# uio-bmi/compairr

Measured on AMD Instinct MI355X. Metric: query sequences/sec for --matrix d=1, 10M-vs-10M CDR3aa, higher is better.
Workload: dtype u64; 1 GPU; synthetic 10M-vs-10M CDR3aa, d=1 substitutions only, V/J matched; queries_total=10000000, queries_this_gpu=10000000, reference_sequences=10000000, matrix_checksum=fc9769626ca2bcf2c84e8473864b8853

## Files before the change

### compairr_amd/csrc/compairr_hip.hip

```cpp
#include "context.h"
#include "kernels_sliced.h"
#include "kernels_rows.h"
#include "kernels_pairs2.h"
#include "select.h"

#include <algorithm>
#include <cmath>
#include <cstdio>
#include <cstdlib>
#include <cstring>
#include <new>
#include <mutex>
#include <string>
#include <thread>
#include <vector>

using namespace cmpr;

std::string &cmpr_create_error()
{
  static thread_local std::string e;
  return e;
}

// ... 225 lines not shown
  invalidate_plan(c);
  c->zob.release();
  c->res2.release(); c->off2.release(); c->cnt2.release();
  c->page_tab.release();
  c->bloom.release(); c->v2.release(); c->j2.release(); c->rep2.release();
  c->rec2.release(); c->voff2.release(); c->bmap2.release();
  for (RefPart &p : c->xparts)
    p.release();
  c->xparts.clear();
  c->stats_acc.release();
  c->tiles.release(); c->qres.release(); c->qv.release(); c->qj.release(); c->qgh.release();
  c->qlen.release(); c->qck.release();
  c->qhins.release(); c->qhdel.release(); c->items.release(); c->cpk.release(); c->qpk.release(); c->slice_items.release(); c->qrec.release();
  c->matrix.release(); c->matrix_f64.release();
  c->pos_buf.release(); c->pos_ctr.release(); c->d_ctab.release(); c->chunks.release(); c->tile_refs.release(); c->small_tiles.release();
  for (uint32_t i = 0; i < cmpr_context::TIME_RING; i++) {
    if (c->ring_k0[i]) (void)hipEventDestroy(c->ring_k0[i]);
    if (c->ring_km[i]) (void)hipEventDestroy(c->ring_km[i]);
    if (c->ring_k1[i]) (void)hipEventDestroy(c->ring_k1[i]);
  }
  if (c->ev_stop) (void)hipEventDestroy(c->ev_stop);
  if (c->ev_usage) (void)hipEventDestroy(c->ev_usage);
  if (c->d_usage) (void)hipFree(c->d_usage);
  if (c->h_usage) (void)hipHostFree(c->h_usage);
  c->arena_a.release();
  c->arena_b.release();
  if (c->stage_host) (void)hipHostFree(c->stage_host);
  if (c->h_sizes) (void)hipHostFree(c->h_sizes);
  for (uint32_t i = 0; i < cmpr_context::NCOPY_EV; i++)
    if (c->ev_copy[i]) (void)hipEventDestroy(c->ev_copy[i]);
// ... 107 lines not shown
    if (value < 1 || value > 2)
      return fail(c, CMPR_EINVAL, "d2_buffers must be 1 or 2");
    if (c->have_ref)
      return fail(c, CMPR_ESTATE, "set d2_buffers before cmpr_set_reference");
    c->d2_buffers = value;
  } else if (n == "chunk_deal") {
    if (value < 0 || value > 1)
      return fail(c, CMPR_EINVAL, "chunk_deal must be 0 (static) or 1 (by a counter)");
    c->chunk_deal = value;
  } else if (n == "narrow_upload") {
    if (value < -1 || value > 1)
      return fail(c, CMPR_EINVAL, "narrow_upload must be -1 (auto), 0 or 1");
    c->narrow_upload = value;
    affects_plan = false;
  } else if (n == "item_wg" || n == "layout_recompute" || n == "layout_timing" || n == "layout_zob_lds" ||
             n == "record_tiles") {
    if (value < 0 || value > (n == "record_tiles" ? 2 : 1))
      return fail(c, CMPR_EINVAL, n + (n == "record_tiles" ? " must be 0, 1 or 2" : " must be 0 or 1"));
    if (n == "record_tiles" && c->have_q)
      return fail(c, CMPR_ESTATE, "set record_tiles before cmpr_set_queries");
    (n == "item_wg" ? c->item_wg : n == "layout_recompute" ? c->layout_recompute :
     n == "layout_zob_lds" ? c->layout_zob_lds : n == "record_tiles" ? c->record_tiles : c->layout_timing) = value;
    affects_plan = false;
  } else if (n == "assume_never_overflows") {
    c->force_no_redo = value != 0;
    c->usage_pending = false;
    affects_plan = false;
  } else if (n == "resolve_blocks_per_cu") {
    if (value < 1 || value > 8)
      return fail(c, CMPR_EINVAL, "resolve_blocks_per_cu must be 1..8");
    c->resolve_blocks_per_cu = value;
  } else if (n == "pos_segments") {
    if (value < 1 || value > 256 || (value & (value - 1)))
      return fail(c, CMPR_EINVAL, "pos_segments must be a power of two, 1..256");
    if (c->have_q)
      return fail(c, CMPR_ESTATE, "set pos_segments before cmpr_set_queries");
    c->pos_segments = value;
// ... 98 lines not shown
  else if (n == "slice_words_log2") *value = c->sliced && c->have_ref ? (int64_t)c->geom.words_log2 : c->slice_words_log2;
  else if (n == "slice_bytes") *value = !c->sliced ? 0 : c->rows ? (int64_t)c->geom.rw_words * ROW_WORD_BYTES : (int64_t)8 << c->geom.words_log2;
  else if (n == "passes") *value = c->npasses;
  else if (n == "chunk_tiles") *value = c->chunk_tiles > 0 ? c->chunk_tiles : 8 * c->waves_per_block;
  else if (n == "waves_per_block") *value = c->plan.valid ? (int64_t)c->plan.nw : c->waves_per_block;
  else if (n == "narrow_upload") *value = c->narrow_upload;
  else if (n == "d2_buffers") *value = c->have_ref && c->d2pairs ? (int64_t)c->geom.nbuf : c->d2_buffers;
  else if (n == "d2_pairs") *value = c->have_ref ? (c->d2pairs ? 1 : 0) : c->d2_pairs;
  else if (n == "chunk_deal") *value = c->chunk_deal;
  else if (n == "layout_upload_us") *value = (int64_t)(c->layout_upload_ms * 1e3);
  else if (n == "layout_tail_us") *value = (int64_t)(c->layout_tail_ms * 1e3);
  else if (n == "layout_total_us") *value = (int64_t)(c->layout_total_ms * 1e3);
  else if (n == "item_wg") *value = c->item_wg;
  else if (n == "layout_recompute") *value = c->layout_recompute;
  else if (n == "layout_timing") *value = c->layout_timing;
  else if (n == "record_tiles") *value = c->have_q ? (c->rec_tiles ? (c->rec_hash ? 1 : 2) : 0) : c->record_tiles;
  else if (n == "layout_keys_us") *value = (int64_t)(c->layout_kernel_ms[0] * 1e3);
  else if (n == "layout_sizes_us") *value = (int64_t)(c->layout_kernel_ms[1] * 1e3);
  else if (n == "layout_scatter_us") *value = (int64_t)(c->layout_kernel_ms[2] * 1e3);
  else if (n == "layout_tiles_us") *value = (int64_t)(c->layout_kernel_ms[3] * 1e3);
  else if (n == "layout_order_us") *value = (int64_t)(c->layout_kernel_ms[4] * 1e3);
  else if (n == "never_overflows") *value = c->never_overflows ? 1 : 0;
  else if (n == "debug") *value = c->debug;
  else if (n == "heavy_threshold") *value = c->heavy_threshold;
  else if (n == "class_anchor") *value = c->sliced && c->have_ref ? (int64_t)c->geom.c0 : c->class_anchor;
  else if (n == "heavy_buckets") {
    *value = 0;
    if (c->sliced && c->have_ref)
      for (uint32_t w = 0; w < HEAVY_WORDS; w++)
        *value += __builtin_popcount(c->ctab[c->geom.off_hv + w]);
// ... 226 lines not shown

static int retire_queries(cmpr_context *c)
{
  HIP_TRY(c, hipSetDevice(c->device));
  if (c->events_valid)
    c->pending_launch = c->ev_k1;
  c->have_q = false;
  c->usage_pending = c->never_overflows = false;
  c->last_without_redo = false;
  c->events_valid = false;
  c->calls = 0;
  invalidate_plan(c);
  return CMPR_OK;
}

int cmpr_settle_previous_launch(cmpr_context *c)
{
  int rc;
  if ((rc = cmpr_wait_previous_launch(c)))
    return rc;
  if (c->async_unchecked || c->async_overflowed) {
    unsigned long long sticky = 0;
    HIP_TRY(c, hipMemcpy(&sticky, c->d_usage + 1, sizeof sticky, hipMemcpyDeviceToHost));
    const bool bad = sticky != 0 || c->async_overflowed;
    if (sticky)
      HIP_TRY(c, hipMemset(c->d_usage + 1, 0, sizeof sticky));
    c->async_unchecked = c->async_overflowed = false;
    if (bad)
      return fail(c, CMPR_ESTATE, "positives buffer overflowed in a launch without redo pass on the previous "
                                  "query set: its result was invalid (cmpr_get_stats was not asked); repeat "
                                  "the call to set the new queries");
  }
  return CMPR_OK;
// ... 11 lines not shown
    std::string why;
    rc = validate_view(c->opt, src.view, why, src.kind == LayoutSource::DEVICE);
    if (rc)
      return fail(c, rc, why);
  } else {
    if (src.nrec && !src.d_records)
      return fail(c, CMPR_EINVAL, "d_records is NULL");
    if (src.nrec && src.n_rep == 0)
      return fail(c, CMPR_EINVAL, "n_repertoires is 0");
    if (src.nrec >= 0xffffffc0ull || src.n_total > 0xffffffffull)
      return fail(c, CMPR_EUNSUPPORTED, "more than 2^32-64 sequences in one set");
  }
  if ((rc = retire_queries(c)))
    return rc;

  src.finish = [c]() -> int {
  int rc;
  const size_t cells = (size_t)c->R1 * c->R2;
  if ((rc = dev_reserve(c, c->matrix, cells))) return rc;
  if (is_f64_score(c->opt)) {
    if ((rc = dev_reserve(c, c->matrix_f64, cells))) return rc;
  } else {
    c->matrix_f64.release();
  }
  {
    const uint64_t per_query = c->rows && c->opt.differences == 2 ? 32 : 4;
    const uint64_t total = c->pos_capacity > 0 ? (uint64_t)c->pos_capacity
                                               : (1u << 20) + per_query * c->n1 /
                                                     (c->routed ? 1ull : (uint64_t)c->work_shard_count);
    const uint64_t S = (uint64_t)c->pos_segments;
    c->pos_cap = (total + S - 1) / S;
    if ((rc = dev_reserve(c, c->pos_buf, S * (c->pos_cap + WAVE)))) return rc;
    if ((rc = dev_reserve(c, c->pos_ctr, 2 * ctr_block_words(S)))) return rc;
    c->ctr_clean = false;
    use_counter_block(c, 0);
    const size_t cells = (size_t)c->R1 * c->R2;
    c->part_stride = (uint32_t)((cells <= PART_CELLS_MAX && !is_f64_score(c->opt) ? cells : 0) + STAT_COUNT);
    if ((rc = dev_reserve(c, c->part, (size_t)NPART * c->part_stride))) return rc;
    HIP_TRY(c, hipMemsetAsync(c->part.p, 0, (size_t)NPART * c->part_stride * sizeof(unsigned long long),
                              c->stream));
  }
  return CMPR_OK;
  };

  if ((rc = cmpr_layout_queries(c, src)))
    return rc;
  if ((rc = make_plan(c))) return rc;
  c->have_q = true;
  return CMPR_OK;
}


static __global__ void __launch_bounds__(WAVE)
sum_part_stats_kernel(const unsigned long long *stats, const unsigned long long *overflow,
                      const unsigned long long *stats2, unsigned long long *acc)
{
  const uint32_t k = threadIdx.x;
// ... 224 lines not shown
  if (!S.will_launch) {
    HIP_TRY(c, hipMemsetAsync(c->ctr_other, 0, S.ctr_blk * sizeof(unsigned long long), st));
    if (c->nparts > 1)
      HIP_TRY(c, hipMemsetAsync(c->stats_acc.p, 0, STAT_COUNT * sizeof(unsigned long long), st));
    if (ev_km)
      HIP_TRY(c, hipEventRecord(ev_km, st));
    c->launches = 0;
    return CMPR_OK;
  }
  const uint32_t np = c->nparts;
  if (np > 1)
    HIP_TRY(c, hipMemsetAsync(c->stats_acc.p, 0, STAT_COUNT * sizeof(unsigned long long), st));
  const bool resolve_pass = S.deferred && !(c->debug & DBG_SKIP_RESOLVE);
  unsigned long long *sticky = (S.redo_kind && !a.with_redo) ? c->d_usage + 1 : nullptr;
  uint32_t launches = 0;
  for (uint32_t k = 0; k < np; k++) {
    ProbeParams P = S.P;
    if (k > 0) {
      use_counter_block(c, c->ctr_cur == c->pos_ctr.p ? 1 : 0);
      const RefPart &rp = c->xparts[k - 1];
      P.bloom = rp.bloom.p;
      P.dir_mask = (uint32_t)(rp.slots - 1);
      P.bmap = S.P.bmap ? rp.bmap.p : nullptr;
      P.rec2 = rp.rec.p;
    }
    P.matrix = a.d_out;
    P.tile_counter = c->d_tile_counter;
    P.deal_ctr = c->d_deal;
    P.stats = c->d_stats;
    P.pair_q = c->pair_q;
    P.pair_h = c->pair_h;
    P.pair_count = c->pair_count;
    P.pair_cap = c->pair_cap;
    if (S.deferred)
      P.pos_ctr = c->ctr_cur;
    if (c->rows && S.deferred)
      P.overflow = c->d_overflow;
    hipLaunchKernelGGL(S.fn, dim3(S.grid), dim3(S.nw * WAVE), S.lds, st, P);
    HIP_TRY(c, hipGetLastError());
    launches += 1;
    if (ev_km && k + 1 == np)
      HIP_TRY(c, hipEventRecord(ev_km, st));
    if (a.track_usage && k == 0)
      HIP_TRY(c, hipMemsetAsync(c->d_usage, 0, sizeof(unsigned long long), st));
    auto reduce_partials = [&]() {
      hipLaunchKernelGGL(reduce_partials_kernel, dim3(P.part_stride), dim3(NPART), 0, st, P,
                         P.part_cells, S.reduce_writes ? 1u : 0u, c->ctr_other,
                         (uint32_t)S.ctr_blk, a.track_usage ? c->d_usage : nullptr, sticky);
    };
    if (!resolve_pass) {
      reduce_partials();
      HIP_TRY(c, hipGetLastError());
    } else {
      hipLaunchKernelGGL(S.rfn, dim3(S.rgrid), dim3(BLOCK_THREADS), S.rlds, st, P);
      reduce_partials();
      HIP_TRY(c, hipGetLastError());
      launches += 1;
      if (a.track_usage && k + 1 == np) {
        HIP_TRY(c, hipMemcpyAsync(c->h_usage, c->d_usage, sizeof(unsigned long long),
// ... 617 lines not shown
```

### compairr_amd/csrc/context.h

```cpp
#ifndef COMPAIRR_AMD_CONTEXT_H
#define COMPAIRR_AMD_CONTEXT_H

#include "../../include/compairr_hip.h"
#include "kernels.h"

#include "select.h"

#include <functional>
#include <map>
#include <set>
#include <string>
#include <vector>

struct SplitMix64 {
  uint64_t s;
  explicit SplitMix64(uint64_t seed) : s(seed) {}
  uint64_t next()
  {
    uint64_t z = (s += 0x9e3779b97f4a7c15ull);
    z = (z ^ (z >> 30)) * 0xbf58476d1ce4e5b9ull;
    z = (z ^ (z >> 27)) * 0x94d049bb133111ebull;
    return z ^ (z >> 31);
  }
};
// ... 40 lines not shown
  uint32_t grid = 0, nw = 0, rgrid = 0;
  size_t   lds = 0, rlds = 0;
};

struct LayoutSource {
  enum Kind { HOST, DEVICE, RECORDS } kind = HOST;
  const cmpr_set_view *view = nullptr;
  const void   *d_records = nullptr;
  uint64_t      nrec = 0;
  uint32_t      n_rep = 0;
  uint64_t      n_total = 0;
  const double *totals = nullptr;
  bool          route = false;
  uint64_t      first_index = 0;
  std::function<int()> finish;
};

struct RouteState {
  bool     valid = false;
  uint64_t n = 0, first_index = 0, total_records = 0;
  uint32_t n_dest = 0, record_bytes = 0;
  unsigned long long counts[64] = {};
  std::vector<double> rep_totals;
  const uint8_t  *res = nullptr;
  const uint64_t *off = nullptr, *cnt = nullptr;
  const uint32_t *v = nullptr, *j = nullptr, *rep = nullptr;
  const uint32_t *mask_lo = nullptr, *mask_hi = nullptr;
  unsigned long long *dest = nullptr;
};

// ... 60 lines not shown
  int64_t debug = 0;
  int64_t slice_words_log2 = -1;
  uint32_t chunk_cap = 0;

  bool                  sliced = false;
  bool                  rows = false;
  uint32_t              npasses = 1;
  SliceGeom             geom{};
  std::vector<uint32_t> ctab;
  DevBuf<uint32_t>      d_ctab;
  DevBuf<uint32_t>      page_tab;
  uint64_t              page_slices = 0;
  DevBuf<Chunk>         chunks;
  DevBuf<cmpr::TileRef> tile_refs;
  DevBuf<uint32_t>      small_tiles;
  uint32_t              nsmall = 0;
  uint32_t              nchunks = 0;

  uint32_t          zpos = 0;
  DevBuf<uint64_t>  zob;

  bool              have_ref = false;
  uint64_t          n2 = 0;
  uint32_t          R2 = 0, longest2 = 0;
  DevBuf<uint8_t>   res2;
  DevBuf<uint64_t>  off2, cnt2, bloom;
  DevBuf<uint32_t>  v2, j2, rep2;
  DevBuf<uint32_t>  bmap2;
  DevBuf<unsigned char> rec2;
  DevBuf<uint32_t>  voff2;
  uint64_t          slots = 0, bloom_words = 0;
  int64_t           part_buckets_log2 = 30;
  uint32_t          nparts = 1;
  uint64_t          part0_n = 0;
  std::vector<RefPart> xparts;
  DevBuf<unsigned long long> stats_acc;

  bool              have_q = false;
  bool              routed = false;
  RouteState        route;
  uint64_t          n1 = 0;
  uint32_t          R1 = 0, ntiles = 0;
  DevBuf<TileDesc>  tiles;
  uint32_t          nmain_tiles = 0;
  DevBuf<uint32_t>  qres, qv, qj;
  DevBuf<uint64_t>  qgh;
  DevBuf<uint64_t>  qhins, qhdel;
  DevBuf<uint16_t>  qlen;
  DevBuf<uint32_t>  qck;
  DevBuf<cmpr::QueryRec> qrec;
  DevBuf<cmpr::ItemRec> items;
  DevBuf<uint32_t>  slice_items;
  DevBuf<cmpr::ResPack> cpk;
  DevBuf<cmpr::ResPack> qpk;
  bool              d2pairs = false;
  int64_t           d2_pairs = -1;
  int64_t           d2_buffers = 1;
  uint64_t          algorithmic_bytes = 0;
  double            max_cell_bound = 0;
  std::vector<double> tot1, tot2;

  DevBuf<unsigned long long> matrix;
  DevBuf<double>             matrix_f64;
  DevBuf<PosEntry>           pos_buf;
  DevBuf<unsigned long long> pos_ctr;
  unsigned long long        *ctr_cur = nullptr, *ctr_other = nullptr;
  bool                       ctr_clean = false;
// ... 5 lines not shown
  bool                       last_without_redo = false;
  bool                       force_no_redo = false;
  bool                       async_unchecked = false, async_overflowed = false;
  hipStream_t                last_stream = nullptr;
  bool                       have_last_stream = false;
  DevArena                   arena_a, arena_b;
  void                      *stage_host = nullptr;
  size_t                     stage_host_bytes = 0;
  int64_t                    narrow_upload = -1;
  hipStream_t                copy_stream = nullptr;
  static const uint32_t      NCOPY_EV = 4;
  hipEvent_t                 ev_copy[NCOPY_EV] = {};
  double                     layout_upload_ms = 0, layout_tail_ms = 0, layout_total_ms = 0;
  int64_t                    item_wg = 1, layout_recompute = 1, layout_timing = 0;
  int64_t                    layout_zob_lds = 1;
  int64_t                    record_tiles = 1;
  bool                       rec_tiles = false;
  bool                       rec_hash = false;
  std::map<std::pair<const void *, size_t>, int> occupancy_seen;
  std::set<std::pair<const void *, size_t>>      lds_raised;
  void                      *h_sizes = nullptr;
  size_t                     h_sizes_bytes = 0;
  hipEvent_t                 ev_layout[6] = {};
  uint32_t                   layout_marks = 0;
  float                      layout_kernel_ms[5] = {};
  StepPlan                   plan;
  unsigned long long        *d_stats = nullptr;
  uint32_t                  *d_tile_counter = nullptr;
  unsigned long long        *d_overflow = nullptr, *d_stats2 = nullptr;
  uint32_t                  *d_tile_counter2 = nullptr;
  unsigned long long        *d_deal = nullptr;
  DevBuf<unsigned long long> part;
  uint32_t                   part_stride = 0;
  const void                *attr_fn2 = nullptr;
  size_t                     attr_lds2 = 0;
  uint64_t                   pos_cap = 0;
  uint32_t                   launches = 0;
  const void                *attr_fn = nullptr;
  size_t                     attr_lds = 0;
// ... 42 lines not shown
  HIP_TRY(c, hipMalloc((void **)&b.p, n * sizeof(T)));
  b.n = n;
  b.cap = n;
  return CMPR_OK;
}

inline int cmpr_wait_previous_launch(cmpr_context *c)
{
  if (c->pending_launch) {
    HIP_TRY(c, hipEventSynchronize(c->pending_launch));
    c->pending_launch = nullptr;
  }
  return CMPR_OK;
}

int cmpr_settle_previous_launch(cmpr_context *c);

template <typename T>
int dev_reserve(cmpr_context *c, DevBuf<T> &b, size_t n)
{
  if (n == 0)
    n = 1;
  if (b.p && b.cap >= n) {
    b.n = n;
    return CMPR_OK;
  }
  b.release();
  const size_t want = n + n / 16;
  HIP_TRY(c, hipMalloc((void **)&b.p, want * sizeof(T)));
  b.n = n;
  b.cap = want;
// ... 61 lines not shown
```

### compairr_amd/csrc/query_layout.hip

```cpp
#include "context.h"
#include "kernels_sliced.h"

#include <hipcub/hipcub.hpp>

#include <algorithm>
#include <atomic>
#include <chrono>
#include <cstdio>
#include <cstdlib>
#include <cstring>
#include <thread>

using namespace cmpr;

namespace {

constexpr uint32_t MAXP = 1 + MAX_CLASS_RES;
constexpr uint32_t FOREIGN_SLICES_LOG2 = 12;

enum : uint32_t { VERR_OFFSETS = 1, VERR_LONG = 2, VERR_REP = 3, VERR_GENE = 4, VERR_COUNT = 5,
                  VERR_RESIDUE = 6, VERR_TOO_LONG = 7, VERR_OFFSETS0 = 8 };

struct SliceTot {
  uint32_t tiles, chunks, small, list;
// ... 1888 lines not shown
        (void)hipStreamSynchronize(c->copy_stream);
        (void)hipStreamSynchronize(c->stream);
      }
    }
  } quiesce{c};
  const cmpr_set_view *const s = src.view;
  const bool from_host = src.kind == LayoutSource::HOST;
  const bool from_records = src.kind == LayoutSource::RECORDS;
  const bool routing = src.route;
  const uint32_t A = (uint32_t)c->opt.alphabet_size;
  const uint32_t Lcap = c->zpos - EXTRA_POSITIONS;
  const uint64_t n = from_records ? src.nrec : s->n;
  const uint32_t n_rep = from_records ? src.n_rep : s->n_repertoires;
  const uint32_t record_bytes = route_record_bytes(Lcap);
  c->route.valid = false;
  uint64_t total = 0;
  if (from_host) {
    total = n ? s->offsets[n] : 0;
  } else if (from_records) {
    total = n * (uint64_t)Lcap;
  }
  const bool total_on_device = src.kind == LayoutSource::DEVICE && n > 0;
  if (n > 0x7fffffffull)
    return fail(c, CMPR_EUNSUPPORTED, "more than 2^31-1 sequences in one set");
  if (!total_on_device && total > 0xffffull * n)
    return fail(c, CMPR_EINVAL, verr_message(VERR_OFFSETS));
  const bool soa_in_arena = src.kind != LayoutSource::DEVICE || n == 0;
  if (!routing) {
    c->n1 = n;
    c->R1 = c->opt.existence ? (uint32_t)(from_records ? src.n_total : n) : n_rep;
// ... 209 lines not shown
    b = 0;
    (void)hipcub::DeviceScan::ExclusiveSum(nullptr, b, (uint32_t *)nullptr, (uint32_t *)nullptr, big, c->stream);
    cub_bytes = std::max(cub_bytes, b);
    b = 0;
    (void)sum64(nullptr, b, nullptr, nullptr, big, c->stream);
    cub_bytes = std::max(cub_bytes, b);
    if (narrow || from_records) {
      hipcub::TransformInputIterator<unsigned long long, Len16To64, const uint16_t *> it(nullptr, Len16To64());
      b = 0;
      (void)hipcub::DeviceScan::ExclusiveScan(nullptr, b, it, (unsigned long long *)nullptr, hipcub::Sum(),
                                              0ull, (int)(n + 1), c->stream);
      cub_bytes = std::max(cub_bytes, b);
    }
  }
  const size_t o_cub = cut.take(cub_bytes + 256);
  if (!(c->arena_a.base && c->arena_a.cap >= cut.used) && (rc = cmpr_wait_previous_launch(c)))
    return rc;
  if ((rc = arena_fit(c, c->arena_a, cut.used))) return rc;
  const auto t_arena_a = std::chrono::steady_clock::now();
  char *const base = c->arena_a.base;
  auto at = [&](size_t off) -> char * { return base + off; };
  HIP_TRY(c, hipMemsetAsync(base, 0, zero_bytes, c->stream));

  QL Q;
  memset(&Q, 0, sizeof Q);
  if (soa_in_arena) {
    Q.res = (const uint8_t *)at(o_res);
    Q.off = (const uint64_t *)at(o_off);
    Q.v = c->opt.ignore_genes ? nullptr : (const uint32_t *)at(o_v);
    Q.j = c->opt.ignore_genes ? nullptr : (const uint32_t *)at(o_j);
    Q.rep = (const uint32_t *)at(o_rep);
    Q.cnt = c->opt.ignore_counts ? nullptr : (const uint64_t *)at(o_cnt);
// ... 438 lines not shown
  }
  const uint64_t cslots = hsums[0], class_chunks = hsums[1];
  if (ntiles * WAVE >= 0xffffffffull)
    return fail(c, CMPR_EUNSUPPORTED, "too many query tiles");
  if (res_words + 9 * WAVE >= 0xffffffffull || cslots + WAVE >= 0xffffffffull)
    return fail(c, CMPR_EUNSUPPORTED, "query set too large for 32-bit residue positions");
  const uint64_t main_chunks = nchunks, main_list = nlist;
  const uint64_t sib_list = hsums[2], sib_chunks = hsums[3];
  nchunks += sib_chunks;
  nlist += sib_list;
  Q.cchunk0 = (uint32_t)nchunks;
  nchunks += class_chunks;
  if (nchunks >= 0x7fffffffull || nlist >= 0xffffffffull)
    return fail(c, CMPR_EUNSUPPORTED, "too many chunks");

  if ((rc = cmpr_settle_previous_launch(c)))
    return rc;

  const size_t slots = (size_t)ntiles * WAVE;
  size_t sort_bytes = 0, small_sort_bytes = 0;
  if (nchunks)
    (void)hipcub::DeviceRadixSort::SortPairsDescending(nullptr, sort_bytes, (uint32_t *)nullptr, (uint32_t *)nullptr,
                                                       (uint32_t *)nullptr, (uint32_t *)nullptr, (int)nchunks, 0, 32,
                                                       c->stream);
  if (nsmall)
    (void)hipcub::DeviceRadixSort::SortPairsDescending(nullptr, small_sort_bytes, (uint32_t *)nullptr,
                                                       (uint32_t *)nullptr, (uint32_t *)nullptr, (uint32_t *)nullptr,
                                                       (int)nsmall, 0, 17, c->stream);
  ArenaCut cb;
  const size_t o_aux = cb.take(std::max<size_t>(Q.recompute ? 1 : slots, 1) * sizeof(QAux));
  const size_t o_chunks_u = cb.take((size_t)nchunks * sizeof(Chunk));
  const size_t o_wk = cb.take(((size_t)nchunks + 1) * sizeof(uint32_t));
  const size_t o_wk2 = cb.take((size_t)nchunks * sizeof(uint32_t));
  const size_t o_ix = cb.take((size_t)nchunks * sizeof(uint32_t));
  const size_t o_ix2 = cb.take((size_t)nchunks * sizeof(uint32_t));
  const size_t o_sort = cb.take(sort_bytes + 256);
  const size_t o_ln = cb.take((size_t)nsmall * sizeof(uint32_t));
  const size_t o_ln2 = cb.take((size_t)nsmall * sizeof(uint32_t));
  const size_t o_sout = cb.take((size_t)nsmall * sizeof(uint32_t));
  const size_t o_ssort = cb.take(small_sort_bytes + 256);
  if ((rc = arena_fit(c, c->arena_b, cb.used))) return rc;
  char *const bb = c->arena_b.base;
  Chunk *const chunks_unsorted = (Chunk *)(bb + o_chunks_u);
  Q.aux = (QAux *)(bb + o_aux);

  c->ntiles = (uint32_t)ntiles;
  c->nchunks = (uint32_t)nchunks;
  c->nsmall = (uint32_t)nsmall;
  if ((rc = dev_reserve(c, c->tiles, (size_t)ntiles))) return rc;
  if ((rc = dev_reserve(c, c->chunks, (size_t)nchunks))) return rc;
  if ((rc = dev_reserve(c, c->tile_refs, (size_t)nlist))) return rc;
  if ((rc = dev_reserve(c, c->small_tiles, (size_t)nsmall))) return rc;
  if ((rc = dev_reserve(c, c->qres, (size_t)res_words + 9 * WAVE))) return rc;
  if ((rc = dev_reserve(c, c->qlen, slots))) return rc;
  if ((rc = dev_reserve(c, c->qrec, slots))) return rc;
  HIP_TRY(c, hipMemsetAsync(c->qres.p + res_words, 0, 9 * WAVE * sizeof(uint32_t), c->stream));
  if (!c->opt.ignore_genes && !c->rows) {
    if ((rc = dev_reserve(c, c->qv, slots))) return rc;
    if ((rc = dev_reserve(c, c->qj, slots))) return rc;
  } else {
    c->qv.release();
    c->qj.release();
  }
  if (!c->opt.ignore_genes || c->rows || (!c->sliced && c->opt.differences == 0)) {
    if ((rc = dev_reserve(c, c->qgh, slots))) return rc;
  } else {
    c->qgh.release();
  }
  if (c->rows) {
    if ((rc = dev_reserve(c, c->qck, slots))) return rc;
  } else {
    c->qck.release();
  }
  if (c->d2pairs) {
    if ((rc = dev_reserve(c, c->qpk, slots))) return rc;
  } else {
    c->qpk.release();
  }
  if (c->rows && c->opt.indels) {
    if ((rc = dev_reserve(c, c->qhins, slots))) return rc;
    if ((rc = dev_reserve(c, c->qhdel, slots))) return rc;
  } else {
    c->qhins.release();
    c->qhdel.release();
  }
  bool pad_items = false;
  if (ngroups) {
    const size_t ni = (size_t)cslots + WAVE;
    if ((rc = dev_reserve(c, c->items, ni))) return rc;
    pad_items = true;
    if (sub2_items) {
      if ((rc = dev_reserve(c, c->cpk, ni))) return rc;
      if ((rc = dev_reserve(c, c->slice_items, 2 * (size_t)nslices_real))) return rc;
      HIP_TRY(c, hipMemsetAsync(c->slice_items.p, 0, 2 * (size_t)nslices_real * sizeof(uint32_t), c->stream));
    } else if (c->d2pairs) {
      if ((rc = dev_reserve(c, c->cpk, ni))) return rc;
      c->slice_items.release();
    } else {
      c->cpk.release();
      c->slice_items.release();
    }
  } else {
    c->items.release();
    c->cpk.release();
    c->slice_items.release();
  }
  const auto t_reserved = std::chrono::steady_clock::now();
  Q.tiles = c->tiles.p;
  Q.chunks = chunks_unsorted;
  Q.tile_refs = c->tile_refs.p;
  Q.small_tiles = c->small_tiles.p;
  Q.cpk = c->cpk.p;
  Q.qpk = c->qpk.p;
  Q.slice_items = (uint2 *)c->slice_items.p;
  Q.qres = c->qres.p; Q.qv = c->qv.p; Q.qj = c->qj.p;
  Q.qck = c->qck.p; Q.qgh = c->qgh.p; Q.qhins = c->qhins.p;
  Q.qhdel = c->qhdel.p; Q.qlen = c->qlen.p; Q.qrec = c->qrec.p;
  Q.items = c->items.p;

  if (pad_items) {
    hipLaunchKernelGGL(item_padding_kernel, dim3(blocks_for(std::max<uint64_t>(ncs, WAVE))), dim3(256), 0, c->stream, Q,
                       cpad, (uint32_t)cslots);
    HIP_TRY(c, hipGetLastError());
  }
  hipLaunchKernelGGL(slices_kernel<1>, dim3((uint32_t)((nslices + SLICES_WG - 1) / SLICES_WG)), dim3(SLICES_WG),
                     slices_lds, c->stream, Q, 0u, slices_lds ? 1u : 0u);
  HIP_TRY(c, hipGetLastError());
  LAYOUT_MARK(2);
  if (n) {
    for (const Range &g : ranges) {
      hipLaunchKernelGGL(scatter_fn, dim3(g.grid), dim3(LAYOUT_WG), scatter_lds, c->stream, Q, g.q0, g.q1, g.row0);
      HIP_TRY(c, hipGetLastError());
    }
  }
  LAYOUT_MARK(3);
  c->rec_tiles = rows_rec;
  c->rec_hash = c->rec_tiles && rec_hash;
  if (ntiles && !c->rec_tiles) {
    const size_t fill_lds = Q.recompute ? (zob_lds ? zob_words * sizeof(uint64_t) : 0) + ctab_bytes : 0;
    const int fo = occupancy_of(c, (const void *)fill_tiles_kernel, 256, fill_lds);
    const uint32_t fgrid = (uint32_t)std::min<uint64_t>((ntiles + 3) / 4, (uint64_t)c->cus * (uint64_t)std::max(fo, 1));
    hipLaunchKernelGGL(fill_tiles_kernel, dim3(fgrid), dim3(256), fill_lds, c->stream, Q, (uint32_t)ntiles);
    HIP_TRY(c, hipGetLastError());
  }
  LAYOUT_MARK(4);
  if (ngroups) {
    hipLaunchKernelGGL(class_chunks_kernel, dim3(blocks_for(ncs)), dim3(256), 0, c->stream, Q);
    HIP_TRY(c, hipGetLastError());
  }
  if (indel_passes) {
    hipLaunchKernelGGL(sibling_fill_kernel, dim3(blocks_for(G)), dim3(256), 0, c->stream, Q, G,
                       sib_lpre, sib_fill, (uint32_t)main_list);
    HIP_TRY(c, hipGetLastError());
    hipLaunchKernelGGL(sibling_write_chunks_kernel, dim3(blocks_for(2 * nslices)), dim3(256), 0,
                       c->stream, Q, sib_cnt, sib_lpre, sib_cpre, (uint32_t)main_list,
                       (uint32_t)main_chunks);
    HIP_TRY(c, hipGetLastError());
  }

  const bool select_share = wstep > 1 && !place_mine;
  if (nchunks && nchunks <= ORDER_MAX && !select_share) {
    uint32_t *wk = (uint32_t *)(bb + o_wk);
    HIP_TRY(c, hipMemsetAsync(wk + nchunks, 0, sizeof(uint32_t), c->stream));
    hipLaunchKernelGGL(chunk_work_kernel, dim3(blocks_for(nchunks)), dim3(256), 0, c->stream, Q,
                       (uint32_t)nchunks, wk, (uint32_t *)nullptr);
    hipLaunchKernelGGL(chunk_order_kernel, dim3(1), dim3(1024), 0, c->stream, Q, (uint32_t)nchunks, wk, c->chunks.p);
    HIP_TRY(c, hipGetLastError());
    c->nchunks = (uint32_t)nchunks;
  } else if (nchunks) {
    uint32_t *wk = (uint32_t *)(bb + o_wk), *wk2 = (uint32_t *)(bb + o_wk2);
    uint32_t *ix = (uint32_t *)(bb + o_ix), *ix2 = (uint32_t *)(bb + o_ix2);
    hipLaunchKernelGGL(chunk_work_kernel, dim3(blocks_for(nchunks)), dim3(256), 0, c->stream, Q,
                       (uint32_t)nchunks, wk, ix);
    HIP_TRY(c, hipGetLastError());
    size_t sb = sort_bytes;
    HIP_TRY(c, hipcub::DeviceRadixSort::SortPairsDescending(bb + o_sort, sb, wk, wk2, ix, ix2, (int)nchunks, 0, 32,
                                                            c->stream));
    uint64_t mine = nchunks;
    const uint32_t *order = ix2;
    Tmp<uint32_t> sel;
    if (select_share) {
      if ((rc = select_mine(c, ix2, (uint32_t)nchunks, sel, mine, [&](unsigned char *flag) {
            hipLaunchKernelGGL(chunk_mine_kernel, dim3(blocks_for(nchunks)), dim3(256), 0, c->stream,
                               chunks_unsorted, ix2, (uint32_t)nchunks, wfirst, wstep, flag);
          })))
        return rc;
      order = sel.b.p;
    }
    if (mine)
      hipLaunchKernelGGL(gather_chunks_kernel, dim3(blocks_for(mine)), dim3(256), 0, c->stream,
                         chunks_unsorted, order, (uint32_t)mine, c->chunks.p);
    HIP_TRY(c, hipGetLastError());
    if (select_share)
      HIP_TRY(c, hipStreamSynchronize(c->stream));
    c->nchunks = (uint32_t)mine;
  }
  if (nsmall) {
    uint32_t *ln = (uint32_t *)(bb + o_ln), *ln2 = (uint32_t *)(bb + o_ln2), *out = (uint32_t *)(bb + o_sout);
    hipLaunchKernelGGL(small_len_kernel, dim3(blocks_for(nsmall)), dim3(256), 0, c->stream, Q,
                       (uint32_t)nsmall, ln);
    HIP_TRY(c, hipGetLastError());
    size_t sb = small_sort_bytes;
    HIP_TRY(c, hipcub::DeviceRadixSort::SortPairsDescending(bb + o_ssort, sb, ln, ln2, c->small_tiles.p, out,
                                                            (int)nsmall, 0, 17, c->stream));
    uint64_t mine = nsmall;
    const uint32_t *keep = out;
    Tmp<uint32_t> sel;
    if (select_share) {
      if ((rc = select_mine(c, out, (uint32_t)nsmall, sel, mine, [&](unsigned char *flag) {
            hipLaunchKernelGGL(small_mine_kernel, dim3(blocks_for(nsmall)), dim3(256), 0, c->stream, Q,
                               out, (uint32_t)nsmall, wfirst, wstep, flag);
          })))
        return rc;
      keep = sel.b.p;
    }
    if (mine)
      HIP_TRY(c, hipMemcpyAsync(c->small_tiles.p, keep, (size_t)mine * sizeof(uint32_t),
                                hipMemcpyDeviceToDevice, c->stream));
    if (select_share)
      HIP_TRY(c, hipStreamSynchronize(c->stream));
    c->nsmall = (uint32_t)mine;
  }
  LAYOUT_MARK(5);
  if (src.finish && (rc = src.finish()))
    return rc;
  HIP_TRY(c, hipStreamSynchronize(c->stream));
  const auto t_end = std::chrono::steady_clock::now();
#undef LAYOUT_MARK
  for (float &x : c->layout_kernel_ms)
    x = 0.0f;
  if (c->layout_marks == 0x3fu) {
    for (int k = 0; k < 5; k++)
      (void)hipEventElapsedTime(&c->layout_kernel_ms[k], c->ev_layout[k], c->ev_layout[k + 1]);
  }
  c->layout_upload_ms = upload_ms;
  c->layout_tail_ms = std::chrono::duration<double, std::milli>(t_end - t_uploaded).count();
  c->layout_total_ms = std::chrono::duration<double, std::milli>(t_end - t_begin).count();
  if (getenv("COMPAIRR_HIP_DEBUG")) {
    auto ms = [](std::chrono::steady_clock::time_point a, std::chrono::steady_clock::time_point b) {
      return std::chrono::duration<double, std::milli>(b - a).count();
    };
// ... 50 lines not shown
```

Measured before the change: 5.790 billion query sequences/s.

## Build tile descriptors into spare buffers early and avoid host wait on previous launch

Query layout now builds tile, chunk, tile-ref and small-tile descriptors into double-buffered spare arrays before settling the previous launch. It then swaps them in. When no scratch buffer would need reallocating, settling the previous launch becomes a stream-side event wait rather than a host synchronize, so layout work for the next batch can queue behind the running matrix kernel. This adds memory for the spare descriptor buffers and more complex lifetime logic, and the usage-counter memset is moved ahead of the first probe launch.

```diff
diff --git a/compairr_amd/csrc/compairr_hip.hip b/compairr_amd/csrc/compairr_hip.hip
--- a/compairr_amd/csrc/compairr_hip.hip
+++ b/compairr_amd/csrc/compairr_hip.hip
@@ -263,6 +263,8 @@
   c->qhins.release(); c->qhdel.release(); c->items.release(); c->cpk.release(); c->qpk.release(); c->slice_items.release(); c->qrec.release();
   c->matrix.release(); c->matrix_f64.release();
   c->pos_buf.release(); c->pos_ctr.release(); c->d_ctab.release(); c->chunks.release(); c->tile_refs.release(); c->small_tiles.release();
+  c->tiles_spare.release(); c->chunks_spare.release(); c->tile_refs_spare.release(); c->small_tiles_spare.release();
+  c->slice_items_spare.release();
   for (uint32_t i = 0; i < cmpr_context::TIME_RING; i++) {
     if (c->ring_k0[i]) (void)hipEventDestroy(c->ring_k0[i]);
     if (c->ring_km[i]) (void)hipEventDestroy(c->ring_km[i]);
@@ -400,13 +402,14 @@
     c->narrow_upload = value;
     affects_plan = false;
   } else if (n == "item_wg" || n == "layout_recompute" || n == "layout_timing" || n == "layout_zob_lds" ||
-             n == "record_tiles") {
+             n == "record_tiles" || n == "early_descriptors") {
     if (value < 0 || value > (n == "record_tiles" ? 2 : 1))
       return fail(c, CMPR_EINVAL, n + (n == "record_tiles" ? " must be 0, 1 or 2" : " must be 0 or 1"));
     if (n == "record_tiles" && c->have_q)
       return fail(c, CMPR_ESTATE, "set record_tiles before cmpr_set_queries");
     (n == "item_wg" ? c->item_wg : n == "layout_recompute" ? c->layout_recompute :
-     n == "layout_zob_lds" ? c->layout_zob_lds : n == "record_tiles" ? c->record_tiles : c->layout_timing) = value;
+     n == "layout_zob_lds" ? c->layout_zob_lds : n == "record_tiles" ? c->record_tiles :
+     n == "early_descriptors" ? c->early_descriptors : c->layout_timing) = value;
     affects_plan = false;
   } else if (n == "assume_never_overflows") {
     c->force_no_redo = value != 0;
@@ -535,6 +538,8 @@
   else if (n == "item_wg") *value = c->item_wg;
   else if (n == "layout_recompute") *value = c->layout_recompute;
   else if (n == "layout_timing") *value = c->layout_timing;
+  else if (n == "early_descriptors") *value = c->early_descriptors;
+  else if (n == "layout_host_wait") *value = c->layout_host_wait ? 1 : 0;
   else if (n == "record_tiles") *value = c->have_q ? (c->rec_tiles ? (c->rec_hash ? 1 : 2) : 0) : c->record_tiles;
   else if (n == "layout_keys_us") *value = (int64_t)(c->layout_kernel_ms[0] * 1e3);
   else if (n == "layout_sizes_us") *value = (int64_t)(c->layout_kernel_ms[1] * 1e3);
@@ -791,9 +796,17 @@
   return CMPR_OK;
 }
 
-int cmpr_settle_previous_launch(cmpr_context *c)
+int cmpr_settle_previous_launch(cmpr_context *c, bool host_needed)
 {
   int rc;
+  if (!host_needed && !c->async_unchecked && !c->async_overflowed) {
+    if (c->pending_launch && hipEventQuery(c->pending_launch) == hipSuccess)
+      c->pending_launch = nullptr;
+    (void)hipGetLastError();
+    if (c->pending_launch)
+      HIP_TRY(c, hipStreamWaitEvent(c->stream, c->pending_launch, 0));
+    return CMPR_OK;
+  }
   if ((rc = cmpr_wait_previous_launch(c)))
     return rc;
   if (c->async_unchecked || c->async_overflowed) {
@@ -835,12 +848,21 @@
   if ((rc = retire_queries(c)))
     return rc;
 
-  src.finish = [c]() -> int {
+  auto scratch = [c](bool *moves) -> int {
   int rc;
+  auto want = [&](auto &b, size_t n) -> int {
+    if (moves) {
+      *moves = *moves || dev_would_grow(b, n);
+      return CMPR_OK;
+    }
+    return dev_reserve(c, b, n);
+  };
   const size_t cells = (size_t)c->R1 * c->R2;
-  if ((rc = dev_reserve(c, c->matrix, cells))) return rc;
+  if ((rc = want(c->matrix, cells))) return rc;
   if (is_f64_score(c->opt)) {
-    if ((rc = dev_reserve(c, c->matrix_f64, cells))) return rc;
+    if ((rc = want(c->matrix_f64, cells))) return rc;
+  } else if (moves) {
+    *moves = *moves || c->matrix_f64.p != nullptr;
   } else {
     c->matrix_f64.release();
   }
@@ -850,18 +872,26 @@
                                                : (1u << 20) + per_query * c->n1 /
                                                      (c->routed ? 1ull : (uint64_t)c->work_shard_count);
     const uint64_t S = (uint64_t)c->pos_segments;
-    c->pos_cap = (total + S - 1) / S;
-    if ((rc = dev_reserve(c, c->pos_buf, S * (c->pos_cap + WAVE)))) return rc;
-    if ((rc = dev_reserve(c, c->pos_ctr, 2 * ctr_block_words(S)))) return rc;
+    const uint64_t pos_cap = (total + S - 1) / S;
+    if ((rc = want(c->pos_buf, S * (pos_cap + WAVE)))) return rc;
+    if ((rc = want(c->pos_ctr, 2 * ctr_block_words(S)))) return rc;
+    const uint32_t part_stride = (uint32_t)((cells <= PART_CELLS_MAX && !is_f64_score(c->opt) ? cells : 0) + STAT_COUNT);
+    if ((rc = want(c->part, (size_t)NPART * part_stride))) return rc;
+    if (moves)
+      return CMPR_OK;
+    c->pos_cap = pos_cap;
     c->ctr_clean = false;
     use_counter_block(c, 0);
-    const size_t cells = (size_t)c->R1 * c->R2;
-    c->part_stride = (uint32_t)((cells <= PART_CELLS_MAX && !is_f64_score(c->opt) ? cells : 0) + STAT_COUNT);
-    if ((rc = dev_reserve(c, c->part, (size_t)NPART * c->part_stride))) return rc;
+    c->part_stride = part_stride;
     HIP_TRY(c, hipMemsetAsync(c->part.p, 0, (size_t)NPART * c->part_stride * sizeof(unsigned long long),
                               c->stream));
   }
   return CMPR_OK;
+  };
+  src.finish = [scratch]() -> int { return scratch(nullptr); };
+  src.finish_reallocates = [scratch]() -> bool {
+    bool moves = false;
+    return scratch(&moves) != CMPR_OK || moves;
   };
 
   if ((rc = cmpr_layout_queries(c, src)))
@@ -1116,6 +1146,8 @@
   const bool resolve_pass = S.deferred && !(c->debug & DBG_SKIP_RESOLVE);
   unsigned long long *sticky = (S.redo_kind && !a.with_redo) ? c->d_usage + 1 : nullptr;
   uint32_t launches = 0;
+  if (a.track_usage)
+    HIP_TRY(c, hipMemsetAsync(c->d_usage, 0, sizeof(unsigned long long), st));
   for (uint32_t k = 0; k < np; k++) {
     ProbeParams P = S.P;
     if (k > 0) {
@@ -1143,8 +1175,6 @@
     launches += 1;
     if (ev_km && k + 1 == np)
       HIP_TRY(c, hipEventRecord(ev_km, st));
-    if (a.track_usage && k == 0)
-      HIP_TRY(c, hipMemsetAsync(c->d_usage, 0, sizeof(unsigned long long), st));
     auto reduce_partials = [&]() {
       hipLaunchKernelGGL(reduce_partials_kernel, dim3(P.part_stride), dim3(NPART), 0, st, P,
                          P.part_cells, S.reduce_writes ? 1u : 0u, c->ctr_other,
diff --git a/compairr_amd/csrc/context.h b/compairr_amd/csrc/context.h
--- a/compairr_amd/csrc/context.h
+++ b/compairr_amd/csrc/context.h
@@ -78,6 +78,7 @@
   bool          route = false;
   uint64_t      first_index = 0;
   std::function<int()> finish;
+  std::function<bool()> finish_reallocates;
 };
 
 struct RouteState {
@@ -168,6 +169,9 @@
   DevBuf<Chunk>         chunks;
   DevBuf<cmpr::TileRef> tile_refs;
   DevBuf<uint32_t>      small_tiles;
+  DevBuf<Chunk>         chunks_spare;
+  DevBuf<cmpr::TileRef> tile_refs_spare;
+  DevBuf<uint32_t>      small_tiles_spare;
   uint32_t              nsmall = 0;
   uint32_t              nchunks = 0;
 
@@ -195,7 +199,7 @@
   RouteState        route;
   uint64_t          n1 = 0;
   uint32_t          R1 = 0, ntiles = 0;
-  DevBuf<TileDesc>  tiles;
+  DevBuf<TileDesc>  tiles, tiles_spare;
   uint32_t          nmain_tiles = 0;
   DevBuf<uint32_t>  qres, qv, qj;
   DevBuf<uint64_t>  qgh;
@@ -205,6 +209,7 @@
   DevBuf<cmpr::QueryRec> qrec;
   DevBuf<cmpr::ItemRec> items;
   DevBuf<uint32_t>  slice_items;
+  DevBuf<uint32_t>  slice_items_spare;
   DevBuf<cmpr::ResPack> cpk;
   DevBuf<cmpr::ResPack> qpk;
   bool              d2pairs = false;
@@ -240,6 +245,7 @@
   double                     layout_upload_ms = 0, layout_tail_ms = 0, layout_total_ms = 0;
   int64_t                    item_wg = 1, layout_recompute = 1, layout_timing = 0;
   int64_t                    layout_zob_lds = 1;
+  int64_t                    early_descriptors = 1;
   int64_t                    record_tiles = 1;
   bool                       rec_tiles = false;
   bool                       rec_hash = false;
@@ -249,6 +255,7 @@
   size_t                     h_sizes_bytes = 0;
   hipEvent_t                 ev_layout[6] = {};
   uint32_t                   layout_marks = 0;
+  bool                       layout_host_wait = false;
   float                      layout_kernel_ms[5] = {};
   StepPlan                   plan;
   unsigned long long        *d_stats = nullptr;
@@ -321,7 +328,13 @@
   return CMPR_OK;
 }
 
-int cmpr_settle_previous_launch(cmpr_context *c);
+int cmpr_settle_previous_launch(cmpr_context *c, bool host_needed = true);
+
+template <typename T>
+inline bool dev_would_grow(const DevBuf<T> &b, size_t n)
+{
+  return !(b.p && b.cap >= (n ? n : 1));
+}
 
 template <typename T>
 int dev_reserve(cmpr_context *c, DevBuf<T> &b, size_t n)
diff --git a/compairr_amd/csrc/query_layout.hip b/compairr_amd/csrc/query_layout.hip
--- a/compairr_amd/csrc/query_layout.hip
+++ b/compairr_amd/csrc/query_layout.hip
@@ -1926,6 +1926,7 @@
   const uint32_t n_rep = from_records ? src.n_rep : s->n_repertoires;
   const uint32_t record_bytes = route_record_bytes(Lcap);
   c->route.valid = false;
+  c->layout_host_wait = false;
   uint64_t total = 0;
   if (from_host) {
     total = n ? s->offsets[n] : 0;
@@ -2165,8 +2166,11 @@
     }
   }
   const size_t o_cub = cut.take(cub_bytes + 256);
-  if (!(c->arena_a.base && c->arena_a.cap >= cut.used) && (rc = cmpr_wait_previous_launch(c)))
-    return rc;
+  if (!(c->arena_a.base && c->arena_a.cap >= cut.used)) {
+    c->layout_host_wait = c->pending_launch != nullptr;
+    if ((rc = cmpr_wait_previous_launch(c)))
+      return rc;
+  }
   if ((rc = arena_fit(c, c->arena_a, cut.used))) return rc;
   const auto t_arena_a = std::chrono::steady_clock::now();
   char *const base = c->arena_a.base;
@@ -2635,8 +2639,8 @@
   if (nchunks >= 0x7fffffffull || nlist >= 0xffffffffull)
     return fail(c, CMPR_EUNSUPPORTED, "too many chunks");
 
-  if ((rc = cmpr_settle_previous_launch(c)))
-    return rc;
+  const bool select_share = wstep > 1 && !place_mine;
+  const bool early = c->early_descriptors != 0 && !select_share;
 
   const size_t slots = (size_t)ntiles * WAVE;
   size_t sort_bytes = 0, small_sort_bytes = 0;
@@ -2665,75 +2669,217 @@
   Chunk *const chunks_unsorted = (Chunk *)(bb + o_chunks_u);
   Q.aux = (QAux *)(bb + o_aux);
 
-  c->ntiles = (uint32_t)ntiles;
-  c->nchunks = (uint32_t)nchunks;
-  c->nsmall = (uint32_t)nsmall;
-  if ((rc = dev_reserve(c, c->tiles, (size_t)ntiles))) return rc;
-  if ((rc = dev_reserve(c, c->chunks, (size_t)nchunks))) return rc;
-  if ((rc = dev_reserve(c, c->tile_refs, (size_t)nlist))) return rc;
-  if ((rc = dev_reserve(c, c->small_tiles, (size_t)nsmall))) return rc;
-  if ((rc = dev_reserve(c, c->qres, (size_t)res_words + 9 * WAVE))) return rc;
-  if ((rc = dev_reserve(c, c->qlen, slots))) return rc;
-  if ((rc = dev_reserve(c, c->qrec, slots))) return rc;
+  struct Descriptors {
+    DevBuf<TileDesc>      &tiles;
+    DevBuf<Chunk>         &chunks;
+    DevBuf<cmpr::TileRef> &tile_refs;
+    DevBuf<uint32_t>      &small_tiles, &slice_items;
+  };
+  Descriptors cur{c->tiles, c->chunks, c->tile_refs, c->small_tiles, c->slice_items};
+  Descriptors spare{c->tiles_spare, c->chunks_spare, c->tile_refs_spare, c->small_tiles_spare, c->slice_items_spare};
+  Descriptors &D = early ? spare : cur;
+  uint64_t chunks_mine = nchunks, small_mine = nsmall;
+  Chunk *chunks_out = nullptr;
+  uint32_t *small_out = nullptr;
+
+  auto descriptors_head = [&]() -> int {
+    int rc;
+    const size_t want[5] = {(size_t)ntiles, (size_t)nchunks, (size_t)nlist, (size_t)nsmall,
+                            sub2_items ? 2 * (size_t)nslices_real : 0};
+    if ((rc = dev_reserve(c, D.tiles, want[0]))) return rc;
+    if ((rc = dev_reserve(c, D.chunks, want[1]))) return rc;
+    if ((rc = dev_reserve(c, D.tile_refs, want[2]))) return rc;
+    if ((rc = dev_reserve(c, D.small_tiles, want[3]))) return rc;
+    if (sub2_items) {
+      if ((rc = dev_reserve(c, D.slice_items, want[4]))) return rc;
+    } else {
+      D.slice_items.release();
+    }
+    if (early) {
+      if (!cur.tiles.p && (rc = dev_reserve(c, cur.tiles, want[0]))) return rc;
+      if (!cur.chunks.p && (rc = dev_reserve(c, cur.chunks, want[1]))) return rc;
+      if (!cur.tile_refs.p && (rc = dev_reserve(c, cur.tile_refs, want[2]))) return rc;
+      if (!cur.small_tiles.p && (rc = dev_reserve(c, cur.small_tiles, want[3]))) return rc;
+      if (sub2_items && !cur.slice_items.p && (rc = dev_reserve(c, cur.slice_items, want[4]))) return rc;
+    }
+    Q.tiles = D.tiles.p;
+    Q.chunks = chunks_unsorted;
+    Q.tile_refs = D.tile_refs.p;
+    Q.small_tiles = D.small_tiles.p;
+    Q.slice_items = (uint2 *)D.slice_items.p;
+    chunks_out = D.chunks.p;
+    small_out = D.small_tiles.p;
+    if (sub2_items)
+      HIP_TRY(c, hipMemsetAsync(D.slice_items.p, 0, 2 * (size_t)nslices_real * sizeof(uint32_t), c->stream));
+    hipLaunchKernelGGL(slices_kernel<1>, dim3((uint32_t)((nslices + SLICES_WG - 1) / SLICES_WG)), dim3(SLICES_WG),
+                       slices_lds, c->stream, Q, 0u, slices_lds ? 1u : 0u);
+    HIP_TRY(c, hipGetLastError());
+    return CMPR_OK;
+  };
+
+  auto descriptors_tail = [&]() -> int {
+    int rc;
+    hipStream_t st = c->stream;
+    if (ngroups) {
+      hipLaunchKernelGGL(class_chunks_kernel, dim3(blocks_for(ncs)), dim3(256), 0, st, Q);
+      HIP_TRY(c, hipGetLastError());
+    }
+    if (indel_passes) {
+      hipLaunchKernelGGL(sibling_fill_kernel, dim3(blocks_for(G)), dim3(256), 0, st, Q, G,
+                         sib_lpre, sib_fill, (uint32_t)main_list);
+      HIP_TRY(c, hipGetLastError());
+      hipLaunchKernelGGL(sibling_write_chunks_kernel, dim3(blocks_for(2 * nslices)), dim3(256), 0,
+                         st, Q, sib_cnt, sib_lpre, sib_cpre, (uint32_t)main_list,
+                         (uint32_t)main_chunks);
+      HIP_TRY(c, hipGetLastError());
+    }
+
+    if (nchunks && nchunks <= ORDER_MAX && !select_share) {
+      uint32_t *wk = (uint32_t *)(bb + o_wk);
+      HIP_TRY(c, hipMemsetAsync(wk + nchunks, 0, sizeof(uint32_t), st));
+      hipLaunchKernelGGL(chunk_work_kernel, dim3(blocks_for(nchunks)), dim3(256), 0, st, Q,
+                         (uint32_t)nchunks, wk, (uint32_t *)nullptr);
+      hipLaunchKernelGGL(chunk_order_kernel, dim3(1), dim3(1024), 0, st, Q, (uint32_t)nchunks, wk, chunks_out);
+      HIP_TRY(c, hipGetLastError());
+    } else if (nchunks) {
+      uint32_t *wk = (uint32_t *)(bb + o_wk), *wk2 = (uint32_t *)(bb + o_wk2);
+      uint32_t *ix = (uint32_t *)(bb + o_ix), *ix2 = (uint32_t *)(bb + o_ix2);
+      hipLaunchKernelGGL(chunk_work_kernel, dim3(blocks_for(nchunks)), dim3(256), 0, st, Q,
+                         (uint32_t)nchunks, wk, ix);
+      HIP_TRY(c, hipGetLastError());
+      size_t sb = sort_bytes;
+      HIP_TRY(c, hipcub::DeviceRadixSort::SortPairsDescending(bb + o_sort, sb, wk, wk2, ix, ix2, (int)nchunks, 0, 32,
+                                                              st));
+      uint64_t mine = nchunks;
+      const uint32_t *order = ix2;
+      Tmp<uint32_t> sel;
+      if (select_share) {
+        if ((rc = select_mine(c, ix2, (uint32_t)nchunks, sel, mine, [&](unsigned char *flag) {
+              hipLaunchKernelGGL(chunk_mine_kernel, dim3(blocks_for(nchunks)), dim3(256), 0, st,
+                                 chunks_unsorted, ix2, (uint32_t)nchunks, wfirst, wstep, flag);
+            })))
+          return rc;
+        order = sel.b.p;
+      }
+      if (mine)
+        hipLaunchKernelGGL(gather_chunks_kernel, dim3(blocks_for(mine)), dim3(256), 0, st,
+                           chunks_unsorted, order, (uint32_t)mine, chunks_out);
+      HIP_TRY(c, hipGetLastError());
+      if (select_share)
+        HIP_TRY(c, hipStreamSynchronize(st));
+      chunks_mine = mine;
+    }
+    if (nsmall) {
+      uint32_t *ln = (uint32_t *)(bb + o_ln), *ln2 = (uint32_t *)(bb + o_ln2), *out = (uint32_t *)(bb + o_sout);
+      hipLaunchKernelGGL(small_len_kernel, dim3(blocks_for(nsmall)), dim3(256), 0, st, Q,
+                         (uint32_t)nsmall, ln);
+      HIP_TRY(c, hipGetLastError());
+      size_t sb = small_sort_bytes;
+      HIP_TRY(c, hipcub::DeviceRadixSort::SortPairsDescending(bb + o_ssort, sb, ln, ln2, small_out, out,
+                                                              (int)nsmall, 0, 17, st));
+      uint64_t mine = nsmall;
+      const uint32_t *keep = out;
+      Tmp<uint32_t> sel;
+      if (select_share) {
+        if ((rc = select_mine(c, out, (uint32_t)nsmall, sel, mine, [&](unsigned char *flag) {
+              hipLaunchKernelGGL(small_mine_kernel, dim3(blocks_for(nsmall)), dim3(256), 0, st, Q,
+                                 out, (uint32_t)nsmall, wfirst, wstep, flag);
+            })))
+          return rc;
+        keep = sel.b.p;
+      }
+      if (mine)
+        HIP_TRY(c, hipMemcpyAsync(small_out, keep, (size_t)mine * sizeof(uint32_t),
+                                  hipMemcpyDeviceToDevice, st));
+      if (select_share)
+        HIP_TRY(c, hipStreamSynchronize(st));
+      small_mine = mine;
+    }
+    return CMPR_OK;
+  };
+
+  if (early) {
+    if ((rc = descriptors_head())) return rc;
+    if ((rc = descriptors_tail())) return rc;
+  }
+
+  bool pad_items = false;
+  auto per_slot = [&](auto want, auto drop) -> int {
+    int rc;
+    if ((rc = want(c->qres, (size_t)res_words + 9 * WAVE))) return rc;
+    if ((rc = want(c->qlen, slots))) return rc;
+    if ((rc = want(c->qrec, slots))) return rc;
+    if (!c->opt.ignore_genes && !c->rows) {
+      if ((rc = want(c->qv, slots))) return rc;
+      if ((rc = want(c->qj, slots))) return rc;
+    } else {
+      drop(c->qv);
+      drop(c->qj);
+    }
+    if (!c->opt.ignore_genes || c->rows || (!c->sliced && c->opt.differences == 0)) {
+      if ((rc = want(c->qgh, slots))) return rc;
+    } else {
+      drop(c->qgh);
+    }
+    if (c->rows) {
+      if ((rc = want(c->qck, slots))) return rc;
+    } else {
+      drop(c->qck);
+    }
+    if (c->d2pairs) {
+      if ((rc = want(c->qpk, slots))) return rc;
+    } else {
+      drop(c->qpk);
+    }
+    if (c->rows && c->opt.indels) {
+      if ((rc = want(c->qhins, slots))) return rc;
+      if ((rc = want(c->qhdel, slots))) return rc;
+    } else {
+      drop(c->qhins);
+      drop(c->qhdel);
+    }
+    if (ngroups) {
+      const size_t ni = (size_t)cslots + WAVE;
+      if ((rc = want(c->items, ni))) return rc;
+      pad_items = true;
+      if (sub2_items || c->d2pairs) {
+        if ((rc = want(c->cpk, ni))) return rc;
+      } else {
+        drop(c->cpk);
+      }
+    } else {
+      drop(c->items);
+      drop(c->cpk);
+    }
+    return CMPR_OK;
+  };
+
+  bool host_needed = true;
+  if (early) {
+    bool moves = false;
+    (void)per_slot([&](auto &b, size_t n) -> int { moves = moves || dev_would_grow(b, n); return CMPR_OK; },
+                   [&](auto &b) { moves = moves || b.p != nullptr; });
+    pad_items = false;
+    host_needed = moves || (src.finish && (!src.finish_reallocates || src.finish_reallocates()));
+  }
+  if (c->pending_launch != nullptr && (host_needed || c->async_unchecked || c->async_overflowed))
+    c->layout_host_wait = true;
+  if ((rc = cmpr_settle_previous_launch(c, host_needed)))
+    return rc;
+  if (early) {
+    std::swap(c->tiles, c->tiles_spare);
+    std::swap(c->chunks, c->chunks_spare);
+    std::swap(c->tile_refs, c->tile_refs_spare);
+    std::swap(c->small_tiles, c->small_tiles_spare);
+    std::swap(c->slice_items, c->slice_items_spare);
+  }
+
+  if ((rc = per_slot([&](auto &b, size_t n) -> int { return dev_reserve(c, b, n); }, [&](auto &b) { b.release(); })))
+    return rc;
   HIP_TRY(c, hipMemsetAsync(c->qres.p + res_words, 0, 9 * WAVE * sizeof(uint32_t), c->stream));
-  if (!c->opt.ignore_genes && !c->rows) {
-    if ((rc = dev_reserve(c, c->qv, slots))) return rc;
-    if ((rc = dev_reserve(c, c->qj, slots))) return rc;
-  } else {
-    c->qv.release();
-    c->qj.release();
-  }
-  if (!c->opt.ignore_genes || c->rows || (!c->sliced && c->opt.differences == 0)) {
-    if ((rc = dev_reserve(c, c->qgh, slots))) return rc;
-  } else {
-    c->qgh.release();
-  }
-  if (c->rows) {
-    if ((rc = dev_reserve(c, c->qck, slots))) return rc;
-  } else {
-    c->qck.release();
-  }
-  if (c->d2pairs) {
-    if ((rc = dev_reserve(c, c->qpk, slots))) return rc;
-  } else {
-    c->qpk.release();
-  }
-  if (c->rows && c->opt.indels) {
-    if ((rc = dev_reserve(c, c->qhins, slots))) return rc;
-    if ((rc = dev_reserve(c, c->qhdel, slots))) return rc;
-  } else {
-    c->qhins.release();
-    c->qhdel.release();
-  }
-  bool pad_items = false;
-  if (ngroups) {
-    const size_t ni = (size_t)cslots + WAVE;
-    if ((rc = dev_reserve(c, c->items, ni))) return rc;
-    pad_items = true;
-    if (sub2_items) {
-      if ((rc = dev_reserve(c, c->cpk, ni))) return rc;
-      if ((rc = dev_reserve(c, c->slice_items, 2 * (size_t)nslices_real))) return rc;
-      HIP_TRY(c, hipMemsetAsync(c->slice_items.p, 0, 2 * (size_t)nslices_real * sizeof(uint32_t), c->stream));
-    } else if (c->d2pairs) {
-      if ((rc = dev_reserve(c, c->cpk, ni))) return rc;
-      c->slice_items.release();
-    } else {
-      c->cpk.release();
-      c->slice_items.release();
-    }
-  } else {
-    c->items.release();
-    c->cpk.release();
-    c->slice_items.release();
-  }
   const auto t_reserved = std::chrono::steady_clock::now();
-  Q.tiles = c->tiles.p;
-  Q.chunks = chunks_unsorted;
-  Q.tile_refs = c->tile_refs.p;
-  Q.small_tiles = c->small_tiles.p;
   Q.cpk = c->cpk.p;
   Q.qpk = c->qpk.p;
-  Q.slice_items = (uint2 *)c->slice_items.p;
   Q.qres = c->qres.p; Q.qv = c->qv.p; Q.qj = c->qj.p;
   Q.qck = c->qck.p; Q.qgh = c->qgh.p; Q.qhins = c->qhins.p;
   Q.qhdel = c->qhdel.p; Q.qlen = c->qlen.p; Q.qrec = c->qrec.p;
@@ -2744,9 +2890,8 @@
                        cpad, (uint32_t)cslots);
     HIP_TRY(c, hipGetLastError());
   }
-  hipLaunchKernelGGL(slices_kernel<1>, dim3((uint32_t)((nslices + SLICES_WG - 1) / SLICES_WG)), dim3(SLICES_WG),
-                     slices_lds, c->stream, Q, 0u, slices_lds ? 1u : 0u);
-  HIP_TRY(c, hipGetLastError());
+  if (!early && (rc = descriptors_head()))
+    return rc;
   LAYOUT_MARK(2);
   if (n) {
     for (const Range &g : ranges) {
@@ -2765,87 +2910,16 @@
     HIP_TRY(c, hipGetLastError());
   }
   LAYOUT_MARK(4);
-  if (ngroups) {
-    hipLaunchKernelGGL(class_chunks_kernel, dim3(blocks_for(ncs)), dim3(256), 0, c->stream, Q);
-    HIP_TRY(c, hipGetLastError());
-  }
-  if (indel_passes) {
-    hipLaunchKernelGGL(sibling_fill_kernel, dim3(blocks_for(G)), dim3(256), 0, c->stream, Q, G,
-                       sib_lpre, sib_fill, (uint32_t)main_list);
-    HIP_TRY(c, hipGetLastError());
-    hipLaunchKernelGGL(sibling_write_chunks_kernel, dim3(blocks_for(2 * nslices)), dim3(256), 0,
-                       c->stream, Q, sib_cnt, sib_lpre, sib_cpre, (uint32_t)main_list,
-                       (uint32_t)main_chunks);
-    HIP_TRY(c, hipGetLastError());
-  }
-
-  const bool select_share = wstep > 1 && !place_mine;
-  if (nchunks && nchunks <= ORDER_MAX && !select_share) {
-    uint32_t *wk = (uint32_t *)(bb + o_wk);
-    HIP_TRY(c, hipMemsetAsync(wk + nchunks, 0, sizeof(uint32_t), c->stream));
-    hipLaunchKernelGGL(chunk_work_kernel, dim3(blocks_for(nchunks)), dim3(256), 0, c->stream, Q,
-                       (uint32_t)nchunks, wk, (uint32_t *)nullptr);
-    hipLaunchKernelGGL(chunk_order_kernel, dim3(1), dim3(1024), 0, c->stream, Q, (uint32_t)nchunks, wk, c->chunks.p);
-    HIP_TRY(c, hipGetLastError());
-    c->nchunks = (uint32_t)nchunks;
-  } else if (nchunks) {
-    uint32_t *wk = (uint32_t *)(bb + o_wk), *wk2 = (uint32_t *)(bb + o_wk2);
-    uint32_t *ix = (uint32_t *)(bb + o_ix), *ix2 = (uint32_t *)(bb + o_ix2);
-    hipLaunchKernelGGL(chunk_work_kernel, dim3(blocks_for(nchunks)), dim3(256), 0, c->stream, Q,
-                       (uint32_t)nchunks, wk, ix);
-    HIP_TRY(c, hipGetLastError());
-    size_t sb = sort_bytes;
-    HIP_TRY(c, hipcub::DeviceRadixSort::SortPairsDescending(bb + o_sort, sb, wk, wk2, ix, ix2, (int)nchunks, 0, 32,
-                                                            c->stream));
-    uint64_t mine = nchunks;
-    const uint32_t *order = ix2;
-    Tmp<uint32_t> sel;
-    if (select_share) {
-      if ((rc = select_mine(c, ix2, (uint32_t)nchunks, sel, mine, [&](unsigned char *flag) {
-            hipLaunchKernelGGL(chunk_mine_kernel, dim3(blocks_for(nchunks)), dim3(256), 0, c->stream,
-                               chunks_unsorted, ix2, (uint32_t)nchunks, wfirst, wstep, flag);
-          })))
-        return rc;
-      order = sel.b.p;
-    }
-    if (mine)
-      hipLaunchKernelGGL(gather_chunks_kernel, dim3(blocks_for(mine)), dim3(256), 0, c->stream,
-                         chunks_unsorted, order, (uint32_t)mine, c->chunks.p);
-    HIP_TRY(c, hipGetLastError());
-    if (select_share)
-      HIP_TRY(c, hipStreamSynchronize(c->stream));
-    c->nchunks = (uint32_t)mine;
-  }
-  if (nsmall) {
-    uint32_t *ln = (uint32_t *)(bb + o_ln), *ln2 = (uint32_t *)(bb + o_ln2), *out = (uint32_t *)(bb + o_sout);
-    hipLaunchKernelGGL(small_len_kernel, dim3(blocks_for(nsmall)), dim3(256), 0, c->stream, Q,
-                       (uint32_t)nsmall, ln);
-    HIP_TRY(c, hipGetLastError());
-    size_t sb = small_sort_bytes;
-    HIP_TRY(c, hipcub::DeviceRadixSort::SortPairsDescending(bb + o_ssort, sb, ln, ln2, c->small_tiles.p, out,
-                                                            (int)nsmall, 0, 17, c->stream));
-    uint64_t mine = nsmall;
-    const uint32_t *keep = out;
-    Tmp<uint32_t> sel;
-    if (select_share) {
-      if ((rc = select_mine(c, out, (uint32_t)nsmall, sel, mine, [&](unsigned char *flag) {
-            hipLaunchKernelGGL(small_mine_kernel, dim3(blocks_for(nsmall)), dim3(256), 0, c->stream, Q,
-                               out, (uint32_t)nsmall, wfirst, wstep, flag);
-          })))
-        return rc;
-      keep = sel.b.p;
-    }
-    if (mine)
-      HIP_TRY(c, hipMemcpyAsync(c->small_tiles.p, keep, (size_t)mine * sizeof(uint32_t),
-                                hipMemcpyDeviceToDevice, c->stream));
-    if (select_share)
-      HIP_TRY(c, hipStreamSynchronize(c->stream));
-    c->nsmall = (uint32_t)mine;
-  }
+  if (!early && (rc = descriptors_tail()))
+    return rc;
   LAYOUT_MARK(5);
   if (src.finish && (rc = src.finish()))
     return rc;
   HIP_TRY(c, hipStreamSynchronize(c->stream));
+  c->pending_launch = nullptr;
+  c->ntiles = (uint32_t)ntiles;
+  c->nchunks = (uint32_t)chunks_mine;
+  c->nsmall = (uint32_t)small_mine;
   const auto t_end = std::chrono::steady_clock::now();
 #undef LAYOUT_MARK
   for (float &x : c->layout_kernel_ms)
```

New measurement: 6.056 billion query sequences/s (median of 6 runs). +4.6%, better.
